# Patoche692/Nexus

Hardware: AMD Instinct MI355X
Metric: Msamples/sec (rays traced/sec) at 1080p, 8-bounce, 1M-tri BVH8; 1/2/4/8 GPU (higher is better)
Workload: dtype f32

## Files before the change

include/nexus/PathTracer.h:

```cpp
#pragma once

#include <cstdint>
#include <vector>

#include "../nexus_hip.h"
#include "Scene.h"

namespace nexus {

class PathTracer {
public:
    PathTracer(uint32_t width, uint32_t height, int device = 0);
    ~PathTracer();
    PathTracer(const PathTracer&) = delete;
    PathTracer& operator=(const PathTracer&) = delete;

    void Reset();
    void FreeDeviceBuffers();
    void ResetFrameNumber();
    void Render(const Scene& scene);
    void OnResize(uint32_t width, uint32_t height);
    void UpdateDeviceScene(const Scene& scene);
    void SetDeviceBlasBuild(Scene& scene, bool enable);
    void SetPixelQuery(uint32_t x, uint32_t y);
    int32_t GetSelectedInstance();
    uint32_t GetFrameNumber() const { return m_FrameNumber; }
    const std::vector<uint32_t>& GetPixelBuffer();
    void SetModes(int rngMode, int compactMode, int conductorMode);
    void SetFramesPerPass(uint32_t frames);
    void SetPassesInFlight(uint32_t passes);
    void SetTailBounce(uint32_t bounce);
    void SetEntryPoints(bool on);
    void SetLightSampling(int mode);
    void SetShadowTransmittance(int mode);
    void SetPixelOrder(int order);
    void SetFeatureBuffers(bool on);
    void ReadFeatureBuffers(std::vector<float>& albedo4, std::vector<float>& normalDepth4);
    void SetAdaptive(const nx_adaptive_params* params);
    uint32_t RenderAdaptive(const Scene& scene, uint32_t maxFrames, uint32_t interval, uint32_t* activePixels = nullptr);
    void ReadSampleCounts(std::vector<uint32_t>& counts);
    static void CreateTileSplitId(void* id128);
    void EnableTileSplit(int worldSize, int rank, const void* id128, uint32_t tileRows = 5);
    void DisableTileSplit();
    bool IsTileSplitRoot() const { return m_TileSplit && m_Rank == 0; }
    nxhip_ctx* GetDeviceContext() const { return m_Ctx; }
// ... 18 lines not shown
```

include/nexus_hip.h:

```cpp
#ifndef NEXUS_HIP_H
#define NEXUS_HIP_H

#include <stddef.h>
#include <stdint.h>

#include "nexus_fmath.h"
#include "nexus_pod.h"

#ifdef __cplusplus
extern "C" {
#endif

typedef struct nxhip_ctx nxhip_ctx;

enum {
    NXHIP_OK = 0,
    NXHIP_ERR_INVALID = 1,
    NXHIP_ERR_HIP = 2,
    NXHIP_ERR_NO_DEVICE = 3,
    NXHIP_ERR_TRAVERSAL = 4,
    NXHIP_ERR_ABI = 5,
    NXHIP_ERR_TIMEOUT = 6
};

// ... 42 lines not shown
enum { NXHIP_SHADOWS_OPAQUE = 0, NXHIP_SHADOWS_TRANSMIT = 1 };
int nxhip_set_shadow_transmittance(nxhip_ctx *ctx, int mode);
int nxhip_set_medium(nxhip_ctx *ctx, const nx_medium *medium);
int nxhip_set_medium_density(nxhip_ctx *ctx, const float *rho, uint32_t nx, uint32_t ny, uint32_t nz);
int nxhip_set_camera(nxhip_ctx *ctx, const nx_camera *camera);
int nxhip_set_render_settings(nxhip_ctx *ctx, const nx_render_settings *settings);
int nxhip_set_modes(nxhip_ctx *ctx, int rngMode, int compactMode, int conductorMode);
int nxhip_set_pixel_map(nxhip_ctx *ctx, const uint32_t *pixelMap, uint32_t localCount);
enum { NXHIP_ORDER_ROWS = 0, NXHIP_ORDER_TILES = 1 };
int nxhip_set_pixel_order(nxhip_ctx *ctx, int order);

int nxhip_set_frames_per_pass(nxhip_ctx *ctx, uint32_t frames);

int nxhip_set_passes_in_flight(nxhip_ctx *ctx, uint32_t passes);

#define NXHIP_TAIL_AUTO 0xffffffffu
int nxhip_set_tail_bounce(nxhip_ctx *ctx, uint32_t bounce);
int nxhip_set_entry_points(nxhip_ctx *ctx, int on);
int nxhip_read_entry_states(nxhip_ctx *ctx, void *out, uint32_t capacityRuns, uint32_t *count);
int nxhip_debug_entry_walks(nxhip_ctx *ctx, uint64_t *count);
int nxhip_debug_read_primary_rays(nxhip_ctx *ctx, float *origin3, float *direction3, uint32_t *pathIndex, uint32_t capacity, uint32_t *count);
int nxhip_debug_pass_flavor(nxhip_ctx *ctx, uint32_t forceGeneral, uint32_t *flavor);
int nxhip_debug_set_thin(nxhip_ctx *ctx, uint32_t lanes, uint32_t iters, int inHooks);
int nxhip_debug_set_thin_pool(nxhip_ctx *ctx, uint32_t slots);
int nxhip_debug_thin_counts(nxhip_ctx *ctx, int32_t counts[2]);
int nxhip_debug_thin_counts_of_pass(nxhip_ctx *ctx, uint32_t bounce, int32_t counts[2]);
int nxhip_debug_ended_rays_of_pass(nxhip_ctx *ctx, uint32_t bounce, int32_t *count);


int nxhip_reset_frame_number(nxhip_ctx *ctx);
// ... 152 lines not shown
```

nexus_amd/capi.py:

```python
import ctypes as C
import os

import numpy as np

from . import pod

_HERE = os.path.dirname(os.path.abspath(__file__))
LIB_PATH = os.environ.get("NEXUS_AMD_LIB") or os.path.join(_HERE, "lib", "libnexus_amd.so")

HIP_SYMBOLS = [
    "nxhip_last_error", "nxhip_device_count", "nxhip_create", "nxhip_destroy", "nxhip_resize", "nxhip_sync",
    "nxhip_upload_blas", "nxhip_clear_blas", "nxhip_set_tlas", "nxhip_set_materials", "nxhip_set_lights",
    "nxhip_upload_texture", "nxhip_clear_textures", "nxhip_set_camera", "nxhip_set_render_settings", "nxhip_set_modes",
    "nxhip_set_pixel_map", "nxhip_set_frames_per_pass", "nxhip_reset_frame_number", "nxhip_set_frame_number", "nxhip_frame_number",
    "nxhip_render_frame", "nxhip_accumulate", "nxhip_render", "nxhip_read_radiance", "nxhip_read_accumulation",
    "nxhip_read_rgba8", "nxhip_write_accumulation", "nxhip_bind_radiance", "nxhip_read_full_accumulation", "nxhip_read_full_rgba8", "nxhip_radiance_device_ptr", "nxhip_accumulation_device_ptr", "nxhip_accumulate_external", "nxhip_compose_tiles",
    "nxhip_read_queue_sizes", "nxhip_set_pixel_query", "nxhip_get_selected_instance", "nxhip_trace_batch",
    "nxhip_trace_shadow_batch", "nxhip_bsdf_sample_batch", "nxhip_bsdf_eval_batch", "nxhip_tex2d_batch", "nxhip_enable_trace_stats", "nxhip_read_trace_stats", "nxhip_enable_kernel_timing",
    "nxhip_read_kernel_times", "nxhip_read_graph_timeline", "nxhip_has_gfx950_code", "nxhip_build_info", "nxhip_set_pixel_order", "nxhip_sync_timeout", "nxhip_debug_set_requeue", "nxhip_debug_thin_counts_of_pass", "nxhip_debug_write_blas_node", "nxhip_rebuild_tlas", "nxhip_read_tlas_index", "nxhip_release_queues", "nxhip_set_device_builder",
    "nxhip_set_instance_transforms", "nxhip_read_tlas", "nxhip_set_passes_in_flight", "nxhip_set_tail_bounce", "nxhip_set_entry_points", "nxhip_read_entry_states", "nxhip_debug_set_thin", "nxhip_debug_set_thin_pool", "nxhip_debug_thin_counts", "nxhip_build_blas", "nxhip_read_blas", "nxhip_set_env_sampling",
    "nxhip_tile_pixel_map", "nxhip_mgpu_unique_id", "nxhip_mgpu_init", "nxhip_mgpu_attach", "nxhip_mgpu_gather", "nxhip_mgpu_read_rgba8",
    "nxhip_mgpu_read_accumulation", "nxhip_mgpu_shutdown", "nxhip_fmath_batch", "nxhip_abi_stamp", "nxhip_check_library", "nxhip_build_blas_batch", "nxhip_read_blas_batch", "nxhip_debug_set_scan_epoch", "nxhip_debug_ended_rays_of_pass", "nxhip_debug_entry_walks", "nxhip_debug_pass_flavor",
    "nxhip_set_aov", "nxhip_read_aov", "nxhip_read_aov_frame", "nxhip_write_aov", "nxhip_denoise", "nxhip_denoise_defaults", "nxhip_read_denoised", "nxhip_read_denoised_rgba8",
    "nxhip_adaptive_defaults", "nxhip_set_adaptive", "nxhip_adaptive_update", "nxhip_render_adaptive", "nxhip_read_sample_counts", "nxhip_read_noise_stats",
    "nxhip_read_block_noise", "nxhip_read_active_map", "nxhip_update_blas", "nxhip_update_blas_device",
    "nxhip_set_light_sampling", "nxhip_read_light_table", "nxhip_light_pick_batch",
    "nxhip_read_env_tables", "nxhip_env_sample_batch", "nxhip_env_eval_batch",
    "nxhip_upload_env_float", "nxhip_read_env_float", "nxhip_read_env_guides",
    "nxhip_set_analytic_lights", "nxhip_analytic_light_sample_batch",
    "nxhip_debug_read_primary_rays",
    "nxhip_set_shadow_transmittance", "nxhip_trace_transmittance_batch",
    "nxhip_set_material_detail", "nxhip_shading_frame_batch",
    "nxhip_set_medium", "nxhip_medium_segment_batch", "nxhip_medium_phase_batch",
    "nxhip_set_medium_density", "nxhip_read_medium_majorants", "nxhip_medium_density_batch", "nxhip_medium_track_batch",
]
HOST_SYMBOLS = [
    "nxh_bvh8_build", "nxh_tlas_build", "nxh_tlas_refit", "nxh_bvh8_refit", "nxh_bvh8_node_count", "nxh_bvh8_prim_count", "nxh_bvh8_nodes",
    "nxh_bvh8_prim_indices", "nxh_bvh8_free", "nxh_bvh2_build", "nxh_mat4_from_trs", "nxh_mat4_invert",
    "nxh_instance_init", "nxh_camera_init", "nxh_loaded_texture_count", "nxh_loaded_texture_info", "nxh_loaded_texture_pixels",
    "nxh_loaded_material_textures", "nxh_loaded_warning_count", "nxh_loaded_warning", "nxh_decode_png", "nxh_write_png", "nxh_write_exr",
    "nxs_scene_add_hdr_map_file", "nxs_renderer_create", "nxs_renderer_destroy", "nxs_renderer_render", "nxs_renderer_reset", "nxs_renderer_on_resize",
    "nxs_renderer_save_screenshot", "nxs_renderer_save_exr", "nxs_renderer_frame_number", "nxs_renderer_megasamples_per_second", "nxs_renderer_device_context",
    "nxs_renderer_set_modes", "nxs_renderer_set_denoise", "nxs_renderer_save_denoised_exr", "nxs_renderer_save_feature_exr", "nxs_pathtracer_set_feature_buffers",
    "nxs_renderer_set_adaptive", "nxs_renderer_render_adaptive", "nxs_renderer_save_sample_count_exr", "nxs_pathtracer_set_adaptive",
    "nxh_load_scene_file", "nxh_loaded_scene_free", "nxh_loaded_mesh_count", "nxh_loaded_mesh_triangle_count", "nxh_loaded_mesh_triangles",
    "nxh_loaded_material_count", "nxh_loaded_materials", "nxh_loaded_instance_count", "nxh_loaded_instances", "nxs_scene_load_file", "nxs_scene_set_instance_transform", "nxs_scene_assign_material", "nxs_scene_set_tlas_refit", "nxs_scene_set_device_tlas", "nxs_scene_update_mesh", "nxs_pathtracer_set_device_blas_build",
    "nxs_last_error", "nxs_scene_create", "nxs_scene_destroy", "nxs_scene_add_material", "nxs_scene_add_texture", "nxs_scene_set_hdr_map",
    "nxs_scene_add_mesh", "nxs_scene_create_instance", "nxs_scene_set_camera", "nxs_scene_set_render_settings", "nxs_scene_update",
    "nxs_scene_light_count", "nxs_scene_instance_count", "nxs_pathtracer_create", "nxs_pathtracer_destroy", "nxs_pathtracer_set_modes", "nxs_pathtracer_set_frames_per_pass", "nxs_pathtracer_set_passes_in_flight", "nxs_pathtracer_set_pixel_order", "nxs_pathtracer_set_entry_points", "nxs_pathtracer_set_light_sampling",
# ... 991 lines not shown
        out = np.zeros((n.value, 40), np.int32)
        if n.value:
            check(self.L.nxhip_read_entry_states(self.h, _ptr(out), n.value, C.byref(n)), "nxhip_read_entry_states")
        return out

    TAIL_AUTO = 0xFFFFFFFF

    def set_tail_bounce(self, bounce):
        self.L.nxhip_set_tail_bounce.argtypes = [C.c_void_p, C.c_uint32]
        check(self.L.nxhip_set_tail_bounce(self.h, bounce), "nxhip_set_tail_bounce")

    def set_passes_in_flight(self, passes):
        self.L.nxhip_set_passes_in_flight.argtypes = [C.c_void_p, C.c_uint32]
        check(self.L.nxhip_set_passes_in_flight(self.h, passes), "nxhip_set_passes_in_flight")

    def set_frames_per_pass(self, frames):
        check(self.L.nxhip_set_frames_per_pass(self.h, frames), "nxhip_set_frames_per_pass")
        self.frames_per_pass = int(frames)

    def write_accumulation(self, accumulation, frame_number):
        a = np.ascontiguousarray(accumulation, dtype=np.float32).reshape(-1, 3)
        assert len(a) == self.local_count
        check(self.L.nxhip_write_accumulation(self.h, _ptr(a), int(frame_number)), "nxhip_write_accumulation")

    def set_aov(self, on=True):
        check(self.L.nxhip_set_aov(self.h, 1 if on else 0), "nxhip_set_aov")

    def read_aov(self):
        a = np.zeros((self.local_count, 4), np.float32)
        n = np.zeros((self.local_count, 4), np.float32)
# ... 236 lines not shown
    n = C.c_uint32(0)
    check(lib().nxhip_tile_pixel_map(width, height, world, rank, tile_rows, 1 if tiled else 0, None, C.byref(n)), "nxhip_tile_pixel_map")
    out = np.zeros(n.value, dtype=np.uint32)
    check(lib().nxhip_tile_pixel_map(width, height, world, rank, tile_rows, 1 if tiled else 0, _ptr(out), C.byref(n)), "nxhip_tile_pixel_map")
    return out


def mgpu_unique_id():
    uid = np.zeros(128, dtype=np.uint8)
    check(lib().nxhip_mgpu_unique_id(_ptr(uid)), "nxhip_mgpu_unique_id")
    return uid.tobytes()


def device_count():
    return int(lib().nxhip_device_count())



def _scheck(rc, what):
    if rc != 0:
        msg = lib().nxs_last_error()
        raise NexusError(f"{what} failed: {msg.decode() if msg else ''}")


class Scene:

    def __init__(self, width, height):
        self.L = lib()
        h = C.c_void_p()
        _scheck(self.L.nxs_scene_create(width, height, C.byref(h)), "nxs_scene_create")
# ... 377 lines not shown
```

nexus_amd/csrc/device/nx_context.h:

```cpp
#pragma once

#include <hip/hip_runtime.h>

#include <memory>
#include <string>
#include <vector>

#include "nexus_hip.h"
#include "nx_device.h"

namespace nxd {

void set_error(const std::string& msg);
bool hip_ok(hipError_t e, const char* what, const char* file, int line);

#define NX_HIP(call)                                                              \
    do {                                                                          \
        if (!::nxd::hip_ok((call), #call, __FILE__, __LINE__)) return NXHIP_ERR_HIP; \
    } while (0)

struct DevBuf {
    void* p = nullptr;
    size_t bytes = 0;
    std::shared_ptr<DevBuf> pool;
// ... 66 lines not shown
    DevBuf thinStates;
    DevBuf thinLists;
    uint32_t scanEpoch = 0;
    DevBuf entryTable;
    uint32_t entryRuns = 0;
    uint64_t entryStamp = 0;
    DevBuf aovAlbedo, aovNormalDepth;
    uint32_t* hostError = nullptr;
    bool errorFresh = false;
    size_t pathCapacity = 0;
    struct GraphInstance {
        hipGraph_t graph = nullptr;
        hipGraphExec_t exec = nullptr;
        int traceBlocks = 0, tailBounce = 0;
        int flavor = 0;
    };
    std::vector<GraphInstance> graphs;
    hipEvent_t done = nullptr, accumulated = nullptr;
    bool awaitingAccumulate = false;
    bool accumulateRecorded = false;
    uint32_t frames = 0, frameLast = 0;
    uint32_t passPixels = 0;
    DeviceState view{};
};

}

struct nxhip_ctx : nxd::PassSlot {
    int device = 0;
    hipStream_t stream2 = nullptr;
    int numCUs = 0;
    std::vector<std::unique_ptr<nxd::PassSlot>> extra;
    uint32_t passesInFlight = 1;
    uint32_t nextSlot = 0;
    std::vector<nxd::PassSlot*> pending;
    nxd::PassSlot* lastRendered = nullptr;

    uint32_t width = 0, height = 0, localCount = 0;
    uint32_t framesPerPass = 1, pathCount = 0;
    size_t queueCapacity = 0;
    size_t radianceBoundCapacity = 0;

    nxd::DeviceState h{};
    bool stateDirty = true;

    std::vector<nxd::BlasHost> blas;
    nxd::DevBuf blasTable;
    nxd::DevBuf tlasTightBoxes;
    nxd::DevBuf tlasNodes, tlasInstIdx, instTrav, instances;
// ... 100 lines not shown
```

nexus_amd/csrc/device/nx_host.h:

```cpp
#pragma once

#include <cstring>
#include <type_traits>
#include <vector>

#include "nx_context.h"

namespace nxd {

const void* trace_kernel_ptr(bool anyHit, bool stats, bool identity = false);
const void* trace_transmit_kernel_ptr(bool stats);
const void* trace_entry_kernel_ptr(bool identity = false);
const void* thin_kernel_ptr();
const void* entry_state_kernel_ptr();
const void* tail_kernel_ptr(bool lightPower, bool analytic = false);
const void* logic_kernel_ptr(int items, bool analytic = false);
const void* shade_kernel_ptr(int type, bool lightPower, bool analytic = false);
const void* shade_scan_kernel_ptr(bool lightPower, bool noMaps = false, bool analytic = false);
const void* count_scan_kernel_ptr();
const void* begin_frame_kernel_ptr();
const void* hook_sizes_kernel_ptr();
const void* generate_kernel_ptr();
const void* accumulate_kernel_ptr();
const void* compose_kernel_ptr();
// ... 238 lines not shown
int alloc_queues(nxhip_ctx* c, size_t n);
bool slot_queues_ready(const nxhip_ctx* c, const PassSlot* q);
int ensure_slot_queues(nxhip_ctx* c, PassSlot* q);
void release_slot_queues(nxhip_ctx* c, PassSlot* q);
void release_denoise_planes(nxhip_ctx* c);
void publish_pixel_set(nxhip_ctx* c);
int set_frame_number_device(nxhip_ctx* c, uint32_t f);
int refresh_shade_inst(nxhip_ctx* c);
bool material_see_through(const nxhip_ctx* c, const nx_material& m);
void refresh_detail_maps(nxhip_ctx* c);
void refresh_see_through(nxhip_ctx* c);
int refresh_updated_blas(nxhip_ctx* c);
int check_scene_ready(nxhip_ctx* c);
int launch_now(nxhip_ctx* c, const Launch& l, hipStream_t stream = nullptr);
int render_pass(nxhip_ctx* c, uint32_t framesArg);
int read_float4_as_float3(nxhip_ctx* c, const void* dev, uint32_t count, float* dst);
int adaptive_restart(nxhip_ctx* c);
int refresh_light_table(nxhip_ctx* c);

}
```

nexus_amd/csrc/device/nxhip_api.hip:

```cpp
#include <algorithm>
#include <cmath>
#include <cstdio>
#include <cstdlib>
#include <chrono>
#include <cstring>
#include <new>
#include <thread>
#include <string>
#include <vector>

#include "nx_host.h"

namespace nxd {

static thread_local std::string g_lastError;

void set_error(const std::string& msg) { g_lastError = msg; }

bool hip_ok(hipError_t e, const char* what, const char* file, int line)
{
    if (e == hipSuccess) return true;
    (void)hipGetLastError();
    char buf[512];
    std::snprintf(buf, sizeof buf, "HIP error %d (%s) in '%s' at %s:%d", (int)e, hipGetErrorString(e), what, file, line);
// ... 351 lines not shown
    if (!out) return fail_invalid("nxhip_create: out is null");
    *out = nullptr;
    if (width == 0 || height == 0) return fail_invalid("nxhip_create: zero-sized viewport");
    if ((uint64_t)width * height > 0x7fffffffull) return fail_invalid("nxhip_create: more than 2^31 pixels");
    if (const int rcLayouts = check_layouts()) return rcLayouts;
    if (nxhip_device_count() <= device || device < 0) {
        set_error("nxhip_create: no such HIP device");
        return NXHIP_ERR_NO_DEVICE;
    }
    NX_HIP(hipSetDevice(device));
    nxhip_ctx* c = new (std::nothrow) nxhip_ctx();
    if (!c) return fail_invalid("nxhip_create: out of host memory");
    c->device = device;
    c->width = width;
    c->height = height;
    int rc = NXHIP_OK;
    do {
        if (stream) c->stream = (hipStream_t)stream;
        else {
            if (!hip_ok(hipStreamCreateWithFlags(&c->stream, hipStreamNonBlocking), "hipStreamCreate", __FILE__, __LINE__)) { rc = NXHIP_ERR_HIP; break; }
            c->ownsStream = true;
        }
        hipDeviceProp_t prop;
        if (!hip_ok(hipGetDeviceProperties(&prop, device), "hipGetDeviceProperties", __FILE__, __LINE__)) { rc = NXHIP_ERR_HIP; break; }
        c->numCUs = prop.multiProcessorCount;

        if (!c->dState.alloc(sizeof(DeviceState)) || !c->counters.alloc(sizeof(Counters)) || !c->frame.alloc(sizeof(FrameState)) ||
            !c->traceStats.alloc(2 * sizeof(TraceStatsDev)) || !c->srgbLut.alloc(256 * sizeof(float))) { rc = NXHIP_ERR_HIP; break; }
        (void)hipMemsetAsync(c->counters.p, 0, sizeof(Counters), c->stream);
        (void)hipMemsetAsync(c->traceStats.p, 0, 2 * sizeof(TraceStatsDev), c->stream);
// ... 61 lines not shown
            }
            if (const char* e = std::getenv("NX_CLOSEST_BLOCKS_PER_CU")) {
                const int n = std::atoi(e);
                if (n >= 1 && n <= 16) { c->traceBlocks = n * c->numCUs; c->traceGridForced = true; }
            }
            if (const char* e = std::getenv("NX_SHADE_BLOCKS_PER_CU")) {
                const int n = std::atoi(e);
                if (n >= 1 && n <= 64) c->shadeBlocksPerCU = n;
            }
            if (const char* e = std::getenv("NX_LOGIC_BLOCKS_PER_CU")) {
                const int n = std::atoi(e);
                if (n >= 1 && n <= 64) c->logicBlocksPerCU = n;
            }
            if (const char* e = std::getenv("NX_THIN_LANES")) { const int n = std::atoi(e); if (n >= 1 && n <= 64) c->h.thinLanes = (uint32_t)n; }
            if (const char* e = std::getenv("NX_THIN_ITERS")) { const int n = std::atoi(e); if (n >= 1 && n <= 4096) c->h.thinIters = (uint32_t)n; }
            if (const char* e = std::getenv("NX_TRACE_BLOCKS_TOTAL")) {
                const int n = std::atoi(e);
                if (n >= 1 && n <= 65536) { c->traceBlocks = c->shadowBlocks = n; c->traceGridForced = true; }
            }
        }
    } while (false);
    if (rc != NXHIP_OK) {
        nxhip_destroy(c);
        return rc;
    }
    *out = c;
    return NXHIP_OK;
}

void nxhip_destroy(nxhip_ctx* c)
// ... 221 lines not shown
```

nexus_amd/csrc/device/nxhip_render.hip:

```cpp
#include <algorithm>
#include <cstdlib>
#include <cstring>
#include <memory>
#include <string>
#include <vector>

#include "nx_host.h"

using namespace nxd;

extern "C" {


int nxhip_reset_frame_number(nxhip_ctx* c)
{
    NX_CHECK_CTX(c);
    NX_HIP(hipSetDevice(c->device));
    const int rc = set_frame_number_device(c, 0);
    if (rc != NXHIP_OK || !c->adaptive) return rc;
    return adaptive_restart(c);
}

int nxhip_set_frame_number(nxhip_ctx* c, uint32_t f)
{
// ... 23 lines not shown
        if (d.roughnessMapId < -1 || (d.roughnessMapId >= 0 && (size_t)d.roughnessMapId >= c->roughnessMaps.size())) return fail_invalid("a material's detail entry refers to a roughness map that has not been uploaded");
    }
    for (const nx_light& l : c->hostLights)
        if (l.type == NX_LIGHT_MESH && l.mesh.meshId >= c->hostInstances.size()) return fail_invalid("a mesh light refers to an instance that does not exist");
    if (c->lightSampling == NXHIP_LIGHTS_POWER) {
        std::vector<bool> seen(c->hostInstances.size(), false);
        for (const nx_light& l : c->hostLights) {
            if (l.type != NX_LIGHT_MESH) continue;
            if (seen[l.mesh.meshId]) return fail_invalid("NXHIP_LIGHTS_POWER: the light list names one instance twice");
            seen[l.mesh.meshId] = true;
        }
    }
    return NXHIP_OK;
}

namespace {

int launch_begin_frame(nxhip_ctx* c, PassSlot* q, uint32_t frames, uint32_t frameLast)
{
    DeviceState* S = q->dState.as<DeviceState>();
    if (++q->scanEpoch >= kScanEpochLimit) {
        if (q->scanStatus.p) NX_HIP(hipMemsetAsync(q->scanStatus.p, 0, q->scanStatus.bytes, q->stream));
        q->scanEpoch = 1;
    }
    NX_HIP(launch_untimed(kernels::begin_frame(), 1, kWideBlockThreads, q->stream, S, frames, frameLast, q->scanEpoch));
    (void)c;
    return NXHIP_OK;
}

uint32_t pass_frames(const nxhip_ctx* c) { return c->passFrames ? c->passFrames : c->framesPerPass; }
double pass_size_in_frames(const nxhip_ctx* c) { return (double)pass_pixels(c) * (double)pass_frames(c) / (1920.0 * 1080.0); }

uint32_t effective_slots(const nxhip_ctx* c)
{
    if (c->timingEnabled || c->statsEnabled || c->radianceBoundCapacity != 0) return 1u;
    return std::min<uint32_t>(c->passesInFlight, (uint32_t)c->extra.size());
}

int trace_blocks(const nxhip_ctx* c, int fullGrid)
{
    if (c->traceGridForced) return fullGrid;
    const int maxPerCU = std::max(1, fullGrid / std::max(1, c->numCUs));
    const int R = (int)std::max(1u, effective_slots(c));
    const bool small = pass_size_in_frames(c) <= 8.0;
    int perCU;
    if (R == 1) perCU = small ? std::min(4, maxPerCU) : maxPerCU;
    else perCU = ((small ? 2 : 3) * maxPerCU + 2 * R - 1) / (2 * R);
    return std::min(std::max(perCU, 1), maxPerCU) * c->numCUs;
}

bool transmit_active(const nxhip_ctx* c) { return c->shadowTransmittance == NXHIP_SHADOWS_TRANSMIT && c->materialsSeeThrough; }
// ... 47 lines not shown
    if (scan_pipeline(c) && !c->materialsNameMaps && !(f & kFlavorEnvMap) && !(f & kFlavorDetail)) f |= kFlavorNoMaps;
    if (c->h.alightCount) f |= kFlavorAnalytic;
    if (transmit_active(c)) f |= kFlavorTransmit;
    if (c->h.mediumOn) f |= kFlavorMedium;
    if (c->h.mediumOn && c->h.mediumRho) f |= kFlavorMediumGrid;
    return f & ~(c->flavorForceGeneral & kFlavorSpecialised);
}

std::vector<std::vector<Launch>> frame_levels(nxhip_ctx* c, PassSlot* q)
{
    const DeviceState* S = q->dState.as<DeviceState>();
    const bool stats = c->statsEnabled;
    const int wide = c->wideBlocks;
    const int wideThreads = kWideBlockThreads;
    std::vector<std::vector<Launch>> levels;
    levels.push_back({make_launch(kernels::generate(), wide, wideThreads, NXHIP_K_GENERATE, S)});
    const bool entry = (pass_flavor(c) & kFlavorEntry) != 0;
    const bool lightPower = (pass_flavor(c) & kFlavorLightPower) != 0;
    const bool identity = (pass_flavor(c) & kFlavorIdentity) != 0, noMaps = (pass_flavor(c) & kFlavorNoMaps) != 0;
    const bool analytic = (pass_flavor(c) & kFlavorAnalytic) != 0;
    const bool transmit = (pass_flavor(c) & kFlavorTransmit) != 0;
    const bool detail = (pass_flavor(c) & kFlavorDetail) != 0;
    const bool medium = (pass_flavor(c) & kFlavorMedium) != 0;
    const bool mediumGrid = (pass_flavor(c) & kFlavorMediumGrid) != 0;
    auto shadow_launch = [&](int shadowBlocksArg, int bounceArg, int thinFlagArg) {
        return transmit ? make_launch(kernels::trace_transmit(stats), shadowBlocksArg, kTraceBlockThreads, NXHIP_K_SHADOW, S, bounceArg)
                        : make_launch(kernels::trace(true, stats, identity), shadowBlocksArg, kTraceBlockThreads, NXHIP_K_SHADOW, S, bounceArg | thinFlagArg);
    };
    const int traceBlocks = trace_blocks(c, c->traceBlocks), shadowBlocks = trace_blocks(c, c->shadowBlocks);
    const int thinFlag = (pass_flavor(c) & kFlavorThin) ? kTraceThinFlag : 0;
// ... 42 lines not shown
            if (bounce == 1) aov_beside(levels.back());
            if (in_use(NX_MAT_CONDUCTOR) && c->h.conductorMode != NX_CONDUCTOR_EXTENDED) {
                levels.push_back({make_launch(kernels::count_scan(), lg, kWideBlockThreads, NXHIP_K_LOGIC, S, bounce, NX_MAT_CONDUCTOR)});
            }
            if (medium) {
                Launch anyHit = shadow_launch(shadowBlocks, bounce, thinFlag);
                anyHit.after = 1;
                levels.push_back({make_launch(kernels::trace(false, stats, identity), traceBlocks, kTraceBlockThreads, NXHIP_K_TRACE, S, bounce | kTraceScanFlag | thinFlag),
                                  make_launch(mediumGrid ? kernels::medium_shadow_grid() : kernels::medium_shadow(), wide, wideThreads, NXHIP_K_SHADE, S, bounce), anyHit});
            } else {
                levels.push_back({make_launch(kernels::trace(false, stats, identity), traceBlocks, kTraceBlockThreads, NXHIP_K_TRACE, S, bounce | kTraceScanFlag | thinFlag),
                                  shadow_launch(shadowBlocks, bounce, thinFlag)});
            }
            thin_level(bounce | kTraceScanFlag);
        }
        return levels;
    }
    thin_level(0);
    const int ob = kShadeBlockOrderedThreads;
    for (int bounce = 1; bounce <= pathLength; bounce++) {
        levels.push_back({make_launch(kernels::logic(c->hdrMap.texels.p ? 1 : 2, analytic), lg, lb, NXHIP_K_LOGIC, S, bounce)});
        if (bounce == 1) aov_beside(levels.back());
        std::vector<Launch> shade;
        if (in_use(NX_MAT_DIFFUSE)) shade.push_back(make_launch(kernels::shade(NX_MAT_DIFFUSE, lightPower, analytic, detail), og, ob, NXHIP_K_SHADE, S, bounce));
        if (in_use(NX_MAT_PLASTIC)) shade.push_back(make_launch(kernels::shade(NX_MAT_PLASTIC, lightPower, analytic, detail), og, ob, NXHIP_K_SHADE, S, bounce));
        if (in_use(NX_MAT_DIELECTRIC)) shade.push_back(make_launch(kernels::shade(NX_MAT_DIELECTRIC, lightPower, analytic, detail), og, ob, NXHIP_K_SHADE, S, bounce));
        if (in_use(NX_MAT_CONDUCTOR) && c->h.conductorMode == NX_CONDUCTOR_EXTENDED) shade.push_back(make_launch(kernels::shade(NX_MAT_CONDUCTOR, lightPower, analytic, detail), og, ob, NXHIP_K_SHADE, S, bounce));
        if (shade.empty()) shade.push_back(make_launch(kernels::shade(NX_MAT_DIFFUSE, lightPower, analytic, detail), og, ob, NXHIP_K_SHADE, S, bounce));
        for (auto& l : shade) levels.push_back({l});
        levels.push_back({make_launch(kernels::trace(false, stats, identity), traceBlocks, kTraceBlockThreads, NXHIP_K_TRACE, S, bounce | thinFlag),
                          shadow_launch(shadowBlocks, bounce, thinFlag)});
        thin_level(bounce);
    }
    return levels;
}

}

int nxd::launch_now(nxhip_ctx* c, const Launch& l, hipStream_t stream)
{
    if (!stream) stream = c->stream;
    void* params[Launch::kMaxArgs];
    l.params(params);
    KernelTimer t;
    t.klass = l.klass;
    auto issue = [&]() -> int {
        if (c->timingEnabled) {
            NX_HIP(hipEventCreate(&t.start));
            NX_HIP(hipEventCreate(&t.stop));
// ... 5 lines not shown
        return NXHIP_OK;
    };
    const int rc = issue();
    if (rc != NXHIP_OK) {
        if (t.start) (void)hipEventDestroy(t.start);
        if (t.stop) (void)hipEventDestroy(t.stop);
    } else if (c->timingEnabled) {
        c->timerPool.push_back(t);
        c->times.launches[l.klass]++;
    }
    return rc;
}

constexpr size_t kMaxGraphInstances = 8;

static int pass_graph(nxhip_ctx* c, PassSlot* q, hipGraphExec_t* execOut)
{
    const int blocks = trace_blocks(c, c->traceBlocks), tail = tail_bounce(c), flavor = pass_flavor(c);
    for (auto& g : q->graphs)
        if (g.traceBlocks == blocks && g.tailBounce == tail && g.flavor == flavor) {
            *execOut = g.exec;
            return NXHIP_OK;
        }
    const bool isMain = q == static_cast<PassSlot*>(c);
    const bool timed = isMain && c->timingMode >= 2;
    if (timed) invalidate_graph(c);
    if (q->graphs.size() >= kMaxGraphInstances) {
        (void)hipStreamSynchronize(q->stream);
        PassSlot::GraphInstance& old = q->graphs.front();
        (void)hipGraphExecDestroy(old.exec);
        (void)hipGraphDestroy(old.graph);
        q->graphs.erase(q->graphs.begin());
    }
    PassSlot::GraphInstance inst;
    inst.traceBlocks = blocks;
    inst.tailBounce = tail;
    inst.flavor = flavor;
    NX_HIP(hipGraphCreate(&inst.graph, 0));
    auto fail = [&](int rc) {
        if (inst.exec) (void)hipGraphExecDestroy(inst.exec);
        if (inst.graph) (void)hipGraphDestroy(inst.graph);
        return rc;
    };
    auto levels = frame_levels(c, q);
    std::vector<hipGraphNode_t> prev;
    for (auto& level : levels) {
        std::vector<hipGraphNode_t> cur;
        std::vector<hipGraphNode_t> done;
        std::vector<bool> hasFollower(level.size(), false);
        for (auto& l : level)
            if (l.after >= 0) hasFollower[(size_t)l.after] = true;
        for (auto& l : level) {
// ... 17 lines not shown
                hipGraphNode_t before, after;
                if (!hip_ok(hipGraphAddEventRecordNode(&before, inst.graph, deps.empty() ? nullptr : deps.data(), deps.size(), t.start), "hipGraphAddEventRecordNode", __FILE__, __LINE__) ||
                    !hip_ok(hipGraphAddKernelNode(&node, inst.graph, &before, 1, &p), "hipGraphAddKernelNode", __FILE__, __LINE__) ||
                    !hip_ok(hipGraphAddEventRecordNode(&after, inst.graph, &node, 1, t.stop), "hipGraphAddEventRecordNode", __FILE__, __LINE__)) return fail(NXHIP_ERR_HIP);
                done.push_back(after);
            } else {
                if (!hip_ok(hipGraphAddKernelNode(&node, inst.graph, deps.empty() ? nullptr : deps.data(), deps.size(), &p), "hipGraphAddKernelNode", __FILE__, __LINE__)) return fail(NXHIP_ERR_HIP);
                done.push_back(node);
            }
        }
        for (size_t i = 0; i < level.size(); i++)
            if (!hasFollower[i]) cur.push_back(done[i]);
        prev.swap(cur);
    }
    if (!hip_ok(hipGraphInstantiate(&inst.exec, inst.graph, nullptr, nullptr, 0), "hipGraphInstantiate", __FILE__, __LINE__)) return fail(NXHIP_ERR_HIP);
    q->graphs.push_back(inst);
    *execOut = inst.exec;
    return NXHIP_OK;
}

static PassSlot* render_slot(nxhip_ctx* c, uint32_t R, uint32_t i) { return R <= 1 ? static_cast<PassSlot*>(c) : c->extra[i].get(); }

static int ensure_entry_table(nxhip_ctx* c, PassSlot* q)
{
    const uint32_t runs = (c->localCount + 63u) / 64u;
    if (q->entryRuns == runs && q->entryTable.p) return NXHIP_OK;
    NX_SYNC_ALL(c);
    NX_ALLOC(q->entryTable, (size_t)std::max(1u, runs) * sizeof(EntryState));
    NX_HIP(hipMemset(q->entryTable.p, 0, (size_t)std::max(1u, runs) * sizeof(EntryState)));
    q->entryRuns = runs;
// ... 78 lines not shown
    if (q->awaitingAccumulate) {
        c->pending.erase(std::remove(c->pending.begin(), c->pending.end(), q), c->pending.end());
        q->awaitingAccumulate = false;
    }
    NX_TRY(launch_begin_frame(c, q, frames, frameLast));
    if (c->entryPoints) NX_TRY(walk_entry_states(c, q));
    c->lastPassFlavor = pass_flavor(c);
    if (c->timingEnabled && c->timingMode == 1) {
        auto levels = frame_levels(c, q);
        for (auto& level : levels)
            for (auto& l : level) NX_TRY(launch_now(c, l));
    } else {
        hipGraphExec_t exec = nullptr;
        NX_TRY(pass_graph(c, q, &exec));
        NX_HIP(hipGraphLaunch(exec, q->stream));
        if (c->timingMode == 3) c->graphTimersPending = true;
        if (c->timingMode == 2) {
            NX_SYNC_ALL(c);
            for (size_t i = 0; i < c->graphTimers.size(); i++) {
                float ms = 0.0f;
                NX_HIP(hipEventElapsedTime(&ms, c->graphTimers[i].start, c->graphTimers[i].stop));
                c->times.ms[c->graphTimers[i].klass] += ms;
                c->times.launches[c->graphTimers[i].klass]++;
            }
        }
    }
    if (!q->hostError) NX_HIP(hipHostMalloc((void**)&q->hostError, sizeof(uint32_t), hipHostMallocDefault));
    NX_HIP(hipMemcpyAsync(q->hostError, &q->frame.as<FrameState>()->errorWord, sizeof(uint32_t), hipMemcpyDeviceToHost, q->stream));
    q->errorFresh = true;
    if (R > 1) NX_HIP(hipEventRecord(q->done, q->stream));
// ... 204 lines not shown
            return NXHIP_ERR_HIP;
        }
        NX_HIP(hipMemset(q->counters.p, 0, sizeof(Counters)));
        FrameState fs{0u, -1, -1, 0u, 0u, {0u, 0u, 0u}};
        NX_HIP(hipMemcpy(q->frame.p, &fs, sizeof fs, hipMemcpyHostToDevice));
        c->extra.push_back(std::move(q));
    }
    for (size_t k = passes > 1 ? passes : 0; k < c->extra.size(); k++)
        if (c->extra[k]->pathCapacity) release_slot_queues(c, c->extra[k].get());
    for (uint32_t k = 0; k < slot_count(c); k++) NX_TRY(ensure_slot_events(slot_at(c, k)));
    c->passesInFlight = passes;
    c->nextSlot = 0;
    c->stateDirty = true;
    return NXHIP_OK;
} NX_CATCH("nxhip_set_passes_in_flight")

int nxhip_set_frames_per_pass(nxhip_ctx* c, uint32_t frames)
{
    NX_CHECK_CTX(c);
    if (frames == 0 || frames > 1024) return fail_invalid("nxhip_set_frames_per_pass: frames must be in [1, 1024]");
    if ((uint64_t)c->localCount * frames > 0x7fffffffull) return fail_invalid("nxhip_set_frames_per_pass: more than 2^31 paths");
    const size_t n = (size_t)std::max<uint32_t>(c->localCount, 1u) * frames;
    if (c->radianceBoundCapacity != 0 && n > c->radianceBoundCapacity)
        return fail_invalid("nxhip_set_frames_per_pass: the bound radiance buffer is too small for this many frames; rebind first");
    if (n > c->queueCapacity) {
        NX_HIP(hipSetDevice(c->device));
        NX_SYNC_ALL(c);
        float4* const boundPtr = c->h.radiance;
        const size_t boundCap = c->radianceBoundCapacity;
        NX_TRY(alloc_queues(c, n));
// ... 207 lines not shown
```

nexus_amd/csrc/host/PathTracer.cpp:

```cpp
#include "nexus/PathTracer.h"

#include <cstring>
#include <stdexcept>
#include <string>

namespace nexus {

namespace {
void Check(int rc, const char* what)
{
    if (rc != NXHIP_OK) throw std::runtime_error(std::string(what) + ": " + nxhip_last_error());
}
}

PathTracer::PathTracer(uint32_t width, uint32_t height, int device) : m_ViewportWidth(width), m_ViewportHeight(height)
{
    Check(nxhip_create(device, width, height, nullptr, &m_Ctx), "nxhip_create");
}

PathTracer::~PathTracer() { nxhip_destroy(m_Ctx); }

void PathTracer::Reset()
{
    if (m_TileSplit) {
// ... 190 lines not shown
        const DensityGrid* g = scene.GetMediumDensity();
        Check(nxhip_set_medium_density(m_Ctx, g ? g->voxels.data() : nullptr, g ? g->nx : 0u, g ? g->ny : 0u, g ? g->nz : 0u), "nxhip_set_medium_density");
        scene.mediumDensityDirty = false;
    }
    const nx_camera cam = Camera::ToDevice(*scene.GetCamera());
    Check(nxhip_set_camera(m_Ctx, &cam), "nxhip_set_camera");
    Check(nxhip_set_render_settings(m_Ctx, reinterpret_cast<const nx_render_settings*>(&scene.GetRenderSettings())), "nxhip_set_render_settings");
}

void PathTracer::SetFramesPerPass(uint32_t frames)
{
    Check(nxhip_set_frames_per_pass(m_Ctx, frames), "nxhip_set_frames_per_pass");
    m_FramesPerPass = frames;
}
void PathTracer::SetPassesInFlight(uint32_t passes) { Check(nxhip_set_passes_in_flight(m_Ctx, passes), "nxhip_set_passes_in_flight"); }
void PathTracer::SetTailBounce(uint32_t bounce) { Check(nxhip_set_tail_bounce(m_Ctx, bounce), "nxhip_set_tail_bounce"); }
void PathTracer::SetEntryPoints(bool on) { Check(nxhip_set_entry_points(m_Ctx, on ? 1 : 0), "nxhip_set_entry_points"); }
void PathTracer::SetLightSampling(int mode) { Check(nxhip_set_light_sampling(m_Ctx, mode), "nxhip_set_light_sampling"); }
void PathTracer::SetShadowTransmittance(int mode) { Check(nxhip_set_shadow_transmittance(m_Ctx, mode), "nxhip_set_shadow_transmittance"); }
void PathTracer::SetPixelOrder(int order)
{
    Check(nxhip_set_pixel_order(m_Ctx, order), "nxhip_set_pixel_order");
    m_PixelOrder = order;
    m_FrameNumber = 0;
}

void PathTracer::SetFeatureBuffers(bool on)
{
    if (on) ResetFrameNumber();
    Check(nxhip_set_aov(m_Ctx, on ? 1 : 0), "nxhip_set_aov");
// ... 108 lines not shown
```

Baseline: 2556.

## Chain graph branches when passes in flight exceed the hardware queue budget

Adds a queue budget, read from GPU_MAX_HW_QUEUES with a default of 4. When several passes are in flight and the number of parallel graph branches would exceed that budget, launches within each level of the HIP graph are serialized into a chain instead of fanning out. The goal is to stop parallel branches from oversubscribing the hardware queues and serializing badly or paying scheduling overhead, at the cost of losing intra-level concurrency. It also adds graph measurement and debug APIs, and keys cached graph instances by shape.

```diff
diff --git a/include/nexus/PathTracer.h b/include/nexus/PathTracer.h
--- a/include/nexus/PathTracer.h
+++ b/include/nexus/PathTracer.h
@@ -29,6 +29,7 @@
     void SetModes(int rngMode, int compactMode, int conductorMode);
     void SetFramesPerPass(uint32_t frames);
     void SetPassesInFlight(uint32_t passes);
+    void SetQueueBudget(int queues);
     void SetTailBounce(uint32_t bounce);
     void SetEntryPoints(bool on);
     void SetLightSampling(int mode);
diff --git a/include/nexus_hip.h b/include/nexus_hip.h
--- a/include/nexus_hip.h
+++ b/include/nexus_hip.h
@@ -80,6 +80,11 @@
 
 int nxhip_set_passes_in_flight(nxhip_ctx *ctx, uint32_t passes);
 
+int nxhip_set_queue_budget(nxhip_ctx *ctx, int queues);
+int nxhip_get_queue_budget(nxhip_ctx *ctx, uint32_t *queues, uint32_t *chained, uint32_t *graphInstances);
+uint32_t nxhip_queue_budget_from_text(const char *text);
+int nxhip_debug_last_graph(nxhip_ctx *ctx, uint32_t *nodes, uint32_t *edges, uint32_t *fanOut);
+
 #define NXHIP_TAIL_AUTO 0xffffffffu
 int nxhip_set_tail_bounce(nxhip_ctx *ctx, uint32_t bounce);
 int nxhip_set_entry_points(nxhip_ctx *ctx, int on);
diff --git a/nexus_amd/capi.py b/nexus_amd/capi.py
--- a/nexus_amd/capi.py
+++ b/nexus_amd/capi.py
@@ -33,6 +33,7 @@
     "nxhip_set_material_detail", "nxhip_shading_frame_batch",
     "nxhip_set_medium", "nxhip_medium_segment_batch", "nxhip_medium_phase_batch",
     "nxhip_set_medium_density", "nxhip_read_medium_majorants", "nxhip_medium_density_batch", "nxhip_medium_track_batch",
+    "nxhip_set_queue_budget", "nxhip_get_queue_budget", "nxhip_queue_budget_from_text", "nxhip_debug_last_graph",
 ]
 HOST_SYMBOLS = [
     "nxh_bvh8_build", "nxh_tlas_build", "nxh_tlas_refit", "nxh_bvh8_refit", "nxh_bvh8_node_count", "nxh_bvh8_prim_count", "nxh_bvh8_nodes",
@@ -1054,6 +1055,22 @@
         self.L.nxhip_set_passes_in_flight.argtypes = [C.c_void_p, C.c_uint32]
         check(self.L.nxhip_set_passes_in_flight(self.h, passes), "nxhip_set_passes_in_flight")
 
+    def set_queue_budget(self, queues):
+        self.L.nxhip_set_queue_budget.argtypes = [C.c_void_p, C.c_int]
+        check(self.L.nxhip_set_queue_budget(self.h, int(queues)), "nxhip_set_queue_budget")
+
+    def queue_budget(self):
+        self.L.nxhip_get_queue_budget.argtypes = [C.c_void_p] + [C.POINTER(C.c_uint32)] * 3
+        q, ch, g = C.c_uint32(0), C.c_uint32(0), C.c_uint32(0)
+        check(self.L.nxhip_get_queue_budget(self.h, C.byref(q), C.byref(ch), C.byref(g)), "nxhip_get_queue_budget")
+        return int(q.value), bool(ch.value), int(g.value)
+
+    def debug_last_graph(self):
+        self.L.nxhip_debug_last_graph.argtypes = [C.c_void_p] + [C.POINTER(C.c_uint32)] * 3
+        n, e, f = C.c_uint32(0), C.c_uint32(0), C.c_uint32(0)
+        check(self.L.nxhip_debug_last_graph(self.h, C.byref(n), C.byref(e), C.byref(f)), "nxhip_debug_last_graph")
+        return int(n.value), int(e.value), int(f.value)
+
     def set_frames_per_pass(self, frames):
         check(self.L.nxhip_set_frames_per_pass(self.h, frames), "nxhip_set_frames_per_pass")
         self.frames_per_pass = int(frames)
@@ -1320,6 +1337,13 @@
 
 def device_count():
     return int(lib().nxhip_device_count())
+
+
+def queue_budget_from_text(text):
+    L = lib()
+    L.nxhip_queue_budget_from_text.argtypes = [C.c_char_p]
+    L.nxhip_queue_budget_from_text.restype = C.c_uint32
+    return int(L.nxhip_queue_budget_from_text(None if text is None else str(text).encode()))
 
 
 
diff --git a/nexus_amd/csrc/device/nx_context.h b/nexus_amd/csrc/device/nx_context.h
--- a/nexus_amd/csrc/device/nx_context.h
+++ b/nexus_amd/csrc/device/nx_context.h
@@ -104,6 +104,8 @@
         hipGraphExec_t exec = nullptr;
         int traceBlocks = 0, tailBounce = 0;
         int flavor = 0;
+        int shape = 0;
+        uint32_t nodes = 0, edges = 0, fanOut = 0;
     };
     std::vector<GraphInstance> graphs;
     hipEvent_t done = nullptr, accumulated = nullptr;
@@ -123,6 +125,9 @@
     std::vector<std::unique_ptr<nxd::PassSlot>> extra;
     uint32_t passesInFlight = 1;
     uint32_t nextSlot = 0;
+    uint32_t queueBudget = 4;
+    int shapeForced = -1;
+    uint32_t lastGraphNodes = 0, lastGraphEdges = 0, lastGraphFanOut = 0;
     std::vector<nxd::PassSlot*> pending;
     nxd::PassSlot* lastRendered = nullptr;
 
diff --git a/nexus_amd/csrc/device/nx_host.h b/nexus_amd/csrc/device/nx_host.h
--- a/nexus_amd/csrc/device/nx_host.h
+++ b/nexus_amd/csrc/device/nx_host.h
@@ -276,6 +276,8 @@
 int check_scene_ready(nxhip_ctx* c);
 int launch_now(nxhip_ctx* c, const Launch& l, hipStream_t stream = nullptr);
 int render_pass(nxhip_ctx* c, uint32_t framesArg);
+uint32_t queue_budget_from_text(const char* text);
+uint32_t queue_budget_from_environment();
 int read_float4_as_float3(nxhip_ctx* c, const void* dev, uint32_t count, float* dst);
 int adaptive_restart(nxhip_ctx* c);
 int refresh_light_table(nxhip_ctx* c);
diff --git a/nexus_amd/csrc/device/nxhip_api.hip b/nexus_amd/csrc/device/nxhip_api.hip
--- a/nexus_amd/csrc/device/nxhip_api.hip
+++ b/nexus_amd/csrc/device/nxhip_api.hip
@@ -389,6 +389,7 @@
     c->device = device;
     c->width = width;
     c->height = height;
+    c->queueBudget = queue_budget_from_environment();
     int rc = NXHIP_OK;
     do {
         if (stream) c->stream = (hipStream_t)stream;
@@ -480,6 +481,7 @@
             }
             if (const char* e = std::getenv("NX_THIN_LANES")) { const int n = std::atoi(e); if (n >= 1 && n <= 64) c->h.thinLanes = (uint32_t)n; }
             if (const char* e = std::getenv("NX_THIN_ITERS")) { const int n = std::atoi(e); if (n >= 1 && n <= 4096) c->h.thinIters = (uint32_t)n; }
+            if (const char* e = std::getenv("NX_GRAPH_SHAPE")) { const int n = std::atoi(e); if (n == 0 || n == 1) c->shapeForced = n; }
             if (const char* e = std::getenv("NX_TRACE_BLOCKS_TOTAL")) {
                 const int n = std::atoi(e);
                 if (n >= 1 && n <= 65536) { c->traceBlocks = c->shadowBlocks = n; c->traceGridForced = true; }
diff --git a/nexus_amd/csrc/device/nxhip_render.hip b/nexus_amd/csrc/device/nxhip_render.hip
--- a/nexus_amd/csrc/device/nxhip_render.hip
+++ b/nexus_amd/csrc/device/nxhip_render.hip
@@ -61,6 +61,15 @@
     return NXHIP_OK;
 }
 
+uint32_t nxd::queue_budget_from_text(const char* text)
+{
+    if (!text || !*text) return 4u;
+    char* end = nullptr;
+    const long n = std::strtol(text, &end, 10);
+    return (*end == '\0' && n >= 1 && n <= 32) ? (uint32_t)n : 4u;
+}
+uint32_t nxd::queue_budget_from_environment() { return queue_budget_from_text(std::getenv("GPU_MAX_HW_QUEUES")); }
+
 namespace {
 
 int launch_begin_frame(nxhip_ctx* c, PassSlot* q, uint32_t frames, uint32_t frameLast)
@@ -82,6 +91,16 @@
 {
     if (c->timingEnabled || c->statsEnabled || c->radianceBoundCapacity != 0) return 1u;
     return std::min<uint32_t>(c->passesInFlight, (uint32_t)c->extra.size());
+}
+
+constexpr int kShapeParallel = 0, kShapeChain = 1;
+constexpr uint32_t kBranchesPerLevel = 2;
+int graph_shape(const nxhip_ctx* c)
+{
+    const uint32_t R = effective_slots(c);
+    if (R <= 1u) return kShapeParallel;
+    if (c->shapeForced >= 0) return c->shapeForced;
+    return R * kBranchesPerLevel + 1u > c->queueBudget ? kShapeChain : kShapeParallel;
 }
 
 int trace_blocks(const nxhip_ctx* c, int fullGrid)
@@ -159,6 +178,15 @@
     const int wide = c->wideBlocks;
     const int wideThreads = kWideBlockThreads;
     std::vector<std::vector<Launch>> levels;
+    const bool chain = graph_shape(c) == kShapeChain;
+    auto shaped = [chain](std::vector<std::vector<Launch>>& ls) {
+        if (chain)
+            for (auto& level : ls)
+                for (size_t k = 1; k < level.size(); k++) {
+                    level[k].after = (int)k - 1;
+                }
+        return std::move(ls);
+    };
     levels.push_back({make_launch(kernels::generate(), wide, wideThreads, NXHIP_K_GENERATE, S)});
     const bool entry = (pass_flavor(c) & kFlavorEntry) != 0;
     const bool lightPower = (pass_flavor(c) & kFlavorLightPower) != 0;
@@ -231,7 +259,7 @@
             }
             thin_level(bounce | kTraceScanFlag);
         }
-        return levels;
+        return shaped(levels);
     }
     thin_level(0);
     const int ob = kShadeBlockOrderedThreads;
@@ -249,7 +277,7 @@
                           shadow_launch(shadowBlocks, bounce, thinFlag)});
         thin_level(bounce);
     }
-    return levels;
+    return shaped(levels);
 }
 
 }
@@ -285,11 +313,26 @@
 
 constexpr size_t kMaxGraphInstances = 8;
 
+static int measure_graph(PassSlot::GraphInstance& inst)
+{
+    size_t nodes = 0, edges = 0;
+    NX_HIP(hipGraphGetNodes(inst.graph, nullptr, &nodes));
+    NX_HIP(hipGraphGetEdges(inst.graph, nullptr, nullptr, &edges));
+    std::vector<hipGraphNode_t> from(edges), to(edges);
+    if (edges) NX_HIP(hipGraphGetEdges(inst.graph, from.data(), to.data(), &edges));
+    size_t widest = 0;
+    for (size_t i = 0; i < edges; i++) widest = std::max(widest, (size_t)std::count(from.begin(), from.begin() + (ptrdiff_t)edges, from[i]));
+    inst.nodes = (uint32_t)nodes;
+    inst.edges = (uint32_t)edges;
+    inst.fanOut = (uint32_t)widest;
+    return NXHIP_OK;
+}
+
 static int pass_graph(nxhip_ctx* c, PassSlot* q, hipGraphExec_t* execOut)
 {
-    const int blocks = trace_blocks(c, c->traceBlocks), tail = tail_bounce(c), flavor = pass_flavor(c);
+    const int blocks = trace_blocks(c, c->traceBlocks), tail = tail_bounce(c), flavor = pass_flavor(c), shape = graph_shape(c);
     for (auto& g : q->graphs)
-        if (g.traceBlocks == blocks && g.tailBounce == tail && g.flavor == flavor) {
+        if (g.traceBlocks == blocks && g.tailBounce == tail && g.flavor == flavor && g.shape == shape) {
             *execOut = g.exec;
             return NXHIP_OK;
         }
@@ -307,6 +350,7 @@
     inst.traceBlocks = blocks;
     inst.tailBounce = tail;
     inst.flavor = flavor;
+    inst.shape = shape;
     NX_HIP(hipGraphCreate(&inst.graph, 0));
     auto fail = [&](int rc) {
         if (inst.exec) (void)hipGraphExecDestroy(inst.exec);
@@ -354,6 +398,7 @@
         prev.swap(cur);
     }
     if (!hip_ok(hipGraphInstantiate(&inst.exec, inst.graph, nullptr, nullptr, 0), "hipGraphInstantiate", __FILE__, __LINE__)) return fail(NXHIP_ERR_HIP);
+    if (const int rcMeasure = measure_graph(inst)) return fail(rcMeasure);
     q->graphs.push_back(inst);
     *execOut = inst.exec;
     return NXHIP_OK;
@@ -462,6 +507,8 @@
         hipGraphExec_t exec = nullptr;
         NX_TRY(pass_graph(c, q, &exec));
         NX_HIP(hipGraphLaunch(exec, q->stream));
+        for (const auto& g : q->graphs)
+            if (g.exec == exec) { c->lastGraphNodes = g.nodes; c->lastGraphEdges = g.edges; c->lastGraphFanOut = g.fanOut; }
         if (c->timingMode == 3) c->graphTimersPending = true;
         if (c->timingMode == 2) {
             NX_SYNC_ALL(c);
@@ -696,6 +743,40 @@
     c->stateDirty = true;
     return NXHIP_OK;
 } NX_CATCH("nxhip_set_passes_in_flight")
+
+int nxhip_set_queue_budget(nxhip_ctx* c, int queues)
+try {
+    NX_CHECK_CTX(c);
+    if (queues < 0 || queues > 32) return fail_invalid("nxhip_set_queue_budget: queues must be 0 (read GPU_MAX_HW_QUEUES) or in [1, 32]");
+    NX_HIP(hipSetDevice(c->device));
+    NX_SYNC_ALL(c);
+    c->queueBudget = queues == 0 ? queue_budget_from_environment() : (uint32_t)queues;
+    return NXHIP_OK;
+} NX_CATCH("nxhip_set_queue_budget")
+
+int nxhip_get_queue_budget(nxhip_ctx* c, uint32_t* queues, uint32_t* chained, uint32_t* graphInstances)
+{
+    NX_CHECK_CTX(c);
+    if (queues) *queues = c->queueBudget;
+    if (chained) *chained = graph_shape(c) == kShapeChain ? 1u : 0u;
+    if (graphInstances) {
+        *graphInstances = 0u;
+        for (uint32_t k = 0; k < slot_count(c); k++) *graphInstances = std::max(*graphInstances, (uint32_t)slot_at(c, k)->graphs.size());
+    }
+    return NXHIP_OK;
+}
+
+uint32_t nxhip_queue_budget_from_text(const char* text) { return queue_budget_from_text(text); }
+
+int nxhip_debug_last_graph(nxhip_ctx* c, uint32_t* nodes, uint32_t* edges, uint32_t* fanOut)
+{
+    NX_DEBUG_HOOK("nxhip_debug_last_graph");
+    NX_CHECK_CTX(c);
+    if (nodes) *nodes = c->lastGraphNodes;
+    if (edges) *edges = c->lastGraphEdges;
+    if (fanOut) *fanOut = c->lastGraphFanOut;
+    return NXHIP_OK;
+}
 
 int nxhip_set_frames_per_pass(nxhip_ctx* c, uint32_t frames)
 {
diff --git a/nexus_amd/csrc/host/PathTracer.cpp b/nexus_amd/csrc/host/PathTracer.cpp
--- a/nexus_amd/csrc/host/PathTracer.cpp
+++ b/nexus_amd/csrc/host/PathTracer.cpp
@@ -228,6 +228,7 @@
     m_FramesPerPass = frames;
 }
 void PathTracer::SetPassesInFlight(uint32_t passes) { Check(nxhip_set_passes_in_flight(m_Ctx, passes), "nxhip_set_passes_in_flight"); }
+void PathTracer::SetQueueBudget(int queues) { Check(nxhip_set_queue_budget(m_Ctx, queues), "nxhip_set_queue_budget"); }
 void PathTracer::SetTailBounce(uint32_t bounce) { Check(nxhip_set_tail_bounce(m_Ctx, bounce), "nxhip_set_tail_bounce"); }
 void PathTracer::SetEntryPoints(bool on) { Check(nxhip_set_entry_points(m_Ctx, on ? 1 : 0), "nxhip_set_entry_points"); }
 void PathTracer::SetLightSampling(int mode) { Check(nxhip_set_light_sampling(m_Ctx, mode), "nxhip_set_light_sampling"); }
```

New measurement: 2733, median of 6. 1.07x the previous value.
